# phecda-xu/FullyCNNSpeechEnhancement

Hardware: AMD Instinct MI355X
Metric: spectrogram frames/sec (CR-CED-16 fwd, 129-bin) (higher is better)
Workload: dtype f32; 1 GPU; CR-CED V3 (16-layer, skip connections) forward, batch 256 per GPU, 129x512, fp32 (BASELINE configs[2]); variant=FullyCNNV3, batch_per_gpu=256, frames=512, bins=129, global_batch=256, fused_available=True, parallelism=batch-shard x1, rccl_world_size=1, weights=random-init (glorot, seed 42), library=rced-hip 0.1 gfx950

## Files before the change

fullycnnspeechenhancement_amd/csrc/kernels_fused_v3_allx6.h:

```cpp
#pragma once

template <class M>
__device__ __forceinline__ void convert_px(unsigned lds0, int i, int f) {
  const unsigned src = lds0 + 4 * (M::kX0Off + 4 + i * kS + f);
  float v[8];
#pragma unroll
  for (int rr = 0; rr < 8; ++rr) v[rr] = lds_ld<float>(src, rr * kS * 4);
  u32x4 h, m, l;
#pragma unroll
  for (int q = 0; q < 4; ++q) {
    const P3 p = split2(v[2 * q], v[2 * q + 1]);
    h[q] = p.h;
    m[q] = p.m;
    l[q] = p.l;
  }
  const unsigned dst = lds0 + 4 * M::kB8Off + (kB8Pad + i * kS + f) * 16;
  lds_st<u32x4>(dst, 0, h);
  lds_st<u32x4>(dst, kB8PlaneBytes, m);
  lds_st<u32x4>(dst, 2 * kB8PlaneBytes, l);
}
template <class M>
__device__ __forceinline__ void convert_x0(unsigned lds0, int wave, int lane) {
  lane = opaque(lane);
  const int tid = wave * 64 + lane;
  convert_px<M>(lds0, tid >> 7, tid & 127);
  if (wave == 7 && lane < kTF) convert_px<M>(lds0, lane, kF - 1);
  const int z = tid - 5 * 64;
  if (z >= 0 && z < 72) {
    const int part = z / 24, rr = z - part * 24;
    const int row = rr < 4 ? rr : rr < 20 ? kB8Pad + kS * ((rr - 4) >> 2) + kF + ((rr - 4) & 3) : kB8Pad + kNPX + (rr - 20);
    lds_st<u32x4>(lds0 + 4 * M::kB8Off + part * kB8PlaneBytes + row * 16, 0, u32x4{0u, 0u, 0u, 0u});
  }
}
static_assert(kB8Rows == kB8Pad + kNPX + 4, "convert_x0 zeroes the planes' pad, gap and trailing rows by this map");

template <class M, int NCH, bool CT2ALL>
__device__ __forceinline__ void fin_run(unsigned ra, unsigned ta, int b0, int b2, int q0, bool ct2first, unsigned zaddr, f32x4 (&acc)[3]) {
  s16x8 a[2][3];
  Parts b[2][3];
  auto ld = [&](auto ic) {
    constexpr int i = decltype(ic)::value, r = i & 1;
    const int q = q0 + i;
    const unsigned ta_i = ta + (unsigned)(64 * q);
#pragma unroll
    for (int p = 0; p < 3; ++p) a[r][p] = lds_ld<s16x8>(ta_i, p * kFinTPart);
    const unsigned ra_i = ra + (unsigned)(16 * (4 * q + (q >> 2)));
    const int bq = b0 + 4 * q;
#pragma unroll
    for (int ct = 0; ct < 3; ++ct) {
      if (ct == 2 && !(CT2ALL || i == 0)) continue;
      const bool ok = ct < 2 ? (unsigned)(bq + 64 * ct) <= 128u : (unsigned)(b2 + 4 * q) <= 128u;
      const unsigned ad = ok ? ra_i + 1088u * ct : zaddr;
      b[r][ct].h = lds_ld<s16x8>(ad, 0);
      b[r][ct].m = lds_ld<s16x8>(ad, kHPlaneBytes);
      b[r][ct].l = lds_ld<s16x8>(ad, 2 * kHPlaneBytes);
    }
  };
  ld(IC<0>{});
  pin();
  static_for<0, NCH>([&](auto ic) {
    constexpr int i = decltype(ic)::value, r = i & 1;
    if constexpr (i + 1 < NCH) ld(IC<i + 1>{});
    pin();
    mma2(a[r], b[r][0], acc[0], a[r], b[r][1], acc[1]);
    if constexpr (CT2ALL) {
      acc[2] = l2x_mma(a[r], b[r][2], acc[2]);
    } else if constexpr (i == 0) {
      if (ct2first) acc[2] = l2x_mma(a[r], b[r][2], acc[2]);
    }
    pin();
  });
}

template <class M>
__device__ __forceinline__ void final_phase_x6(const Params& P, unsigned lds0, int wave, int lane, int utt, int t0, const XStage& xnext, float* x0 DET_ARG) {
  DET_BEGIN();
  lane = opaque(lane);
  const int n = lane & 15, kq = lane >> 4;
  const f32x4 zero4 = {0.f, 0.f, 0.f, 0.f};
  float* yt = P.y + ((size_t)utt * P.T + t0) * kF;
  const int nfr = P.T - t0 < kTF ? P.T - t0 : kTF;
  xstage_store(xnext, x0, wave * 64 + lane);
  {
    const int fi = n >> 2, j0 = n & 3;
    const int b0 = 16 * j0 - 64 + kq;
    const int b2 = j0 == 0 ? b0 + 128 : 0x40000000;
    const unsigned ra = lds0 + 4 * M::kB8Off + (unsigned)((kHFr * fi + 17 * j0 - 68 + kq) * 16);
    const unsigned ta = lds0 + 4 * M::kFinTOff + (unsigned)((kq - n + 15) * 16);
    const unsigned zaddr = lds0 + 4 * M::kB8Off + kHZeroRow * 16;
    f32x4 acc[3] = {zero4, zero4, zero4};
    if (wave < 4) {
      fin_run<M, 4, true>(ra, ta, b0, b2, 4 * wave, false, zaddr, acc);
    } else {
      const int run = 11 - wave;
      fin_run<M, 5, false>(ra, ta, b0, b2, 16 + 5 * (run - 4), run == 4, zaddr, acc);
    }
    const unsigned scr = lds0 + (unsigned)M::finscr(wave, 0) + (unsigned)lane * 16u;
#pragma unroll
    for (int ct = 0; ct < 3; ++ct) lds_st<f32x4>(scr, ct * M::kPlaneBytes, acc[ct]);
  }
  DET(8);
  __syncthreads();
  DET(9);
  if (wave < 3) {
    const unsigned scr = lds0 + (unsigned)(M::finscr(0, 0) + wave * M::kPlaneBytes) + (unsigned)lane * 16u;
    f32x4 v = lds_ld<f32x4>(scr, 0);
#pragma unroll
    for (int w = 1; w < kWaves; ++w) v += lds_ld<f32x4>(scr, M::finscr(w, 0) - M::finscr(0, 0));
    v += f32x4{P.fin_bias, P.fin_bias, P.fin_bias, P.fin_bias};
    const int fi = n >> 2;
    if (wave < 2) {
      const int f0 = 16 * (4 * wave + (n & 3)) + 4 * kq;
      if (fi < nfr) {
        *reinterpret_cast<f32x4_u*>(yt + fi * kF + f0) = v;
        store_wait_state();
      }
    } else if (kq == 0 && (n & 3) == 0 && fi < nfr) {
      yt[fi * kF + kF - 1] = v.x;
    }
  }
  DET(10);
  convert_x0<M>(lds0, wave, lane);
  DET(11);
  __syncthreads();
  DET(12);
}
```

fullycnnspeechenhancement_amd/csrc/kernels_fused_v3_l23.h:

```cpp
#pragma once
#ifndef RCED_T_A2REG
#define RCED_T_A2REG 3
#endif
#ifndef RCED_T_PRIO
#define RCED_T_PRIO 1
#endif
#ifndef RCED_T_TAILW
#define RCED_T_TAILW 4
#endif
#ifndef RCED_T_A3D
#define RCED_T_A3D 1
#endif
#ifndef RCED_T_SGB
#define RCED_T_SGB 1
#endif
#ifndef RCED_T_L1PF
#define RCED_T_L1PF 1
#endif
#ifndef RCED_T_EXP
#define RCED_T_EXP 0
#endif
#if (RCED_T_EXP != 0 || RCED_X6_EXP != 0) && !defined(RCED_TIMING_ONLY)
#error "RCED_T_EXP / RCED_X6_EXP builds compute wrong results: timing experiments only (tools/mkexp.sh ... -DRCED_TIMING_ONLY -DRCED_T_EXP=...)"
#endif

template <int CTRL>
__device__ __forceinline__ float dpp0(float v) {
  return __builtin_bit_cast(float, __builtin_amdgcn_update_dpp(0, __builtin_bit_cast(int, v), CTRL, 0xf, 0xf, true));
}
template <int S>
__device__ __forceinline__ void tap_add(float p, float& oP, float& oC, float& oN) {
  if constexpr (S == 0) {
    oC += p;
  } else if constexpr (S > 0) {
    oC += dpp0<0x110 + S>(p);
    oN += dpp0<0x100 + 16 - S>(p);
  } else {
    oC += dpp0<0x100 - S>(p);
    oP += dpp0<0x110 + 16 + S>(p);
  }
}
__device__ __forceinline__ void mma2(const s16x8 (&a0)[3], const Parts& b0, f32x4& c0, const s16x8 (&a1)[3], const Parts& b1, f32x4& c1) {
  c0 = mfma32(a0[1], b0.m, c0);
  c1 = mfma32(a1[1], b1.m, c1);
  c0 = mfma32(a0[2], b0.h, c0);
  c1 = mfma32(a1[2], b1.h, c1);
  c0 = mfma32(a0[0], b0.l, c0);
  c1 = mfma32(a1[0], b1.l, c1);
  c0 = mfma32(a0[1], b0.h, c0);
  c1 = mfma32(a1[1], b1.h, c1);
  c0 = mfma32(a0[0], b0.m, c0);
  c1 = mfma32(a1[0], b1.m, c1);
  c0 = mfma32(a0[0], b0.h, c0);
  c1 = mfma32(a1[0], b1.h, c1);
}
template <int NM, int NV, int ND = 0>
__device__ __forceinline__ void interleave() {
#if RCED_T_SGB
#pragma unroll
  for (int i = 0; i < NM; ++i) {
    __builtin_amdgcn_sched_group_barrier(0x008, 1, 0);
    if (ND > 0) __builtin_amdgcn_sched_group_barrier(0x100, ND, 0);
    __builtin_amdgcn_sched_group_barrier(0x002, NV, 0);
  }
#endif
}
template <int J>
__device__ __forceinline__ void shift_add(f32x4 pj, float& p0, float& p1, float& c0, float& c1, float& n0, float& n1) {
  if (RCED_T_EXP & 1) {
    c0 += pj.x;
    c1 += pj.z;
    return;
  }
  tap_add<4 - 2 * J>(pj.x, p0, c0, n0);
  if constexpr (2 * J + 1 < 9) tap_add<3 - 2 * J>(pj.y, p0, c0, n0);
  tap_add<4 - 2 * J>(pj.z, p1, c1, n1);
  if constexpr (2 * J + 1 < 9) tap_add<3 - 2 * J>(pj.w, p1, c1, n1);
}

template <class M>
struct MapTag {
  typedef M type;
};
template <class M>
constexpr int tail_off() {
  if constexpr (M::kAllX6) return M::kTailOff;
  else return 0;
}
template <class M, bool LAST, class Sp, class Dma1>
__device__ __forceinline__ void layer23(const Params& P, const Lane& L, unsigned lds0, unsigned wbase, const A2Regs& A, int blk, int wave,
                                        unsigned tag, f32x2 (&sk1)[5], f32x2 (&sk2)[5], Sp sp, Dma1 dma1 DET_ARG) {
  DET_BEGIN();
  const bool right = wave >= 4;
  const int fr = wave & 3;
  const unsigned a2 = wbase + L.scr, a3 = a2 + kG2 * 4;
  const f32x4 sh2[2] = {lds_ld<f32x4>(wbase + L.kq16, kG2Data * 4), lds_ld<f32x4>(wbase + L.kq16, (kG2Data + 16) * 4)};
  const f32x2 sh3 = lds_ld<f32x2>(wbase + (L.kq16 >> 1), (kG2 + kW3TData) * 4);
  const f32x4 zero4 = {0.f, 0.f, 0.f, 0.f};
  const f32x2 zero2 = {0.f, 0.f};
  Parts b2[2];
  s16x8 a2m0[3][3];
  if constexpr (RCED_T_A2REG == 3) {
#pragma unroll
    for (int c = 0; c < 3; ++c)
#pragma unroll
      for (int q = 0; q < 3; ++q) a2m0[c][q] = lds_ld<s16x8>(a2, ((2 * c) * 3 + q) * 1024);
  }
  s16x8 a2r[2][2][3];
  unsigned rdc = L.rd2c;
  f32x4 acc2[2][2];
  u32x4 b3h[2], b3m[2], b3l[2];
  s16x8 a3r[RCED_T_A3D + 1][3];
  f32x4 pj[2][2], p4[2] = {zero4, zero4};
  float w0 = -0.f, w1 = -0.f, x0 = -0.f, x1 = -0.f, y0 = -0.f, y1 = -0.f, z0 = -0.f, z1 = -0.f;
  f32x2 hold = zero2;

  auto ldX = [&](auto tc, auto cc) {
    constexpr int t = decltype(tc)::value, c = decltype(cc)::value;
    if ((RCED_T_EXP & 8) && (c > 0 || t > 1)) return;
    Parts& b = b2[(3 * t + c) & 1];
#pragma unroll
    for (int mt = (RCED_T_A2REG == 3 ? 1 : RCED_T_A2REG); mt < 2; ++mt)
#pragma unroll
      for (int q = 0; q < 3; ++q) a2r[(3 * t + c) & 1][mt][q] = lds_ld<s16x8>(a2, ((2 * c + mt) * 3 + q) * 1024);
    if constexpr (c < 2) {
      constexpr int off = t * M::kTileB18 + (M::kAllX6 ? 32 : 64) * c;
      b.h = lds_ld<s16x8>(L.rd2m, off);
      b.m = lds_ld<s16x8>(L.rd2m, off + M::kPlaneBytes);
      b.l = lds_ld<s16x8>(L.rd2m, off + 2 * M::kPlaneBytes);
    } else {
      u32x4 h, m, l;
#pragma unroll
      for (int i = 0; i < 4; ++i) {
        h[i] = lds_ld<unsigned>(rdc, 4 * i);
        m[i] = lds_ld<unsigned>(rdc, 4 * i + M::kPlaneBytes);
        l[i] = lds_ld<unsigned>(rdc, 4 * i + 2 * M::kPlaneBytes);
      }
      b.h = __builtin_bit_cast(s16x8, h);
      b.m = __builtin_bit_cast(s16x8, m);
      b.l = __builtin_bit_cast(s16x8, l);
      rdc += L.rd2cs;
    }
  };
  auto doX = [&](auto tc, auto cc) {
    constexpr int t = decltype(tc)::value, c = decltype(cc)::value, r = (3 * t + c) & 1, u = t & 1;
    if constexpr (c == 0) {
      acc2[u][0] = sh2[0];
      acc2[u][1] = sh2[1];
    }
    mma2(RCED_T_A2REG == 3 ? a2m0[c] : RCED_T_A2REG >= 1 ? A.a[0][c] : a2r[r][0], b2[r], acc2[u][0], RCED_T_A2REG == 2 ? A.a[1][c] : a2r[r][1], b2[r], acc2[u][1]);
  };
  auto split_piece = [&](auto tc, auto qc) {
    constexpr int t = decltype(tc)::value, q = decltype(qc)::value, u = t & 1, mt = q >> 1;
    float v0 = relu1((q & 1) ? acc2[u][mt].z : acc2[u][mt].x), v1 = relu1((q & 1) ? acc2[u][mt].w : acc2[u][mt].y);
    if constexpr (t == 4) {
      const bool ok = vbit(L, kVN0);
      v0 = ok ? v0 : 0.f;
      v1 = ok ? v1 : 0.f;
    }
    P3 p;
    if (RCED_T_EXP & 4) {
      p.h = __builtin_bit_cast(unsigned, v0);
      p.m = __builtin_bit_cast(unsigned, v1);
      p.l = p.h;
    } else {
      p = split2(v0, v1);
    }
    b3h[u][q] = p.h;
    b3m[u][q] = p.m;
    b3l[u][q] = p.l;
  };
  auto ldY = [&](auto jc, auto parc) {
    constexpr int j = decltype(jc)::value, r = (j + decltype(parc)::value) % (RCED_T_A3D + 1);
    if ((RCED_T_EXP & 2) && j > 1) return;
#pragma unroll
    for (int q = 0; q < 3; ++q) a3r[r][q] = lds_ld<s16x8>(a3, (((RCED_T_EXP & 32) ? 0 : j) * 3 + ((RCED_T_EXP & 64) ? 0 : q)) * 1024);
  };
  auto doY = [&](auto uc, auto jc, auto parc) {
    constexpr int u = decltype(uc)::value, j = decltype(jc)::value, r = (j + decltype(parc)::value) % (RCED_T_A3D + 1);
    Parts b;
    b.h = __builtin_bit_cast(s16x8, b3h[u]);
    b.m = __builtin_bit_cast(s16x8, b3m[u]);
    b.l = __builtin_bit_cast(s16x8, b3l[u]);
    if constexpr (j == kL3MT - 1) p4[u] = l2x_mma(a3r[r], b, zero4);
    else pj[u][j & 1] = l2x_mma(a3r[r], b, zero4);
  };
  auto doYY = [&](auto jc, auto parc) {
    constexpr int j = decltype(jc)::value, r = (j + decltype(parc)::value) % (RCED_T_A3D + 1);
    Parts ba, bb;
    ba.h = __builtin_bit_cast(s16x8, b3h[0]);
    ba.m = __builtin_bit_cast(s16x8, b3m[0]);
    ba.l = __builtin_bit_cast(s16x8, b3l[0]);
    bb.h = __builtin_bit_cast(s16x8, b3h[1]);
    bb.m = __builtin_bit_cast(s16x8, b3m[1]);
    bb.l = __builtin_bit_cast(s16x8, b3l[1]);
    f32x4 ca = zero4, cb = zero4;
    mma2(a3r[r], ba, ca, a3r[r], bb, cb);
    if constexpr (j == kL3MT - 1) {
      p4[0] = ca;
      p4[1] = cb;
    } else {
      pj[0][j & 1] = ca;
      pj[1][j & 1] = cb;
    }
  };
  auto finish = [&](auto tc, float s0, float s1) {
    constexpr int t = decltype(tc)::value;
    f32x2 v = {relu1(s0 + sh3.x), relu1(s1 + sh3.y)};
    if constexpr (LAST) {
      v += sk1[t];
    } else {
      v += blk == 3 ? sk2[t] : zero2;
      sk1[t] = blk == 0 ? v : sk1[t];
      sk2[t] = blk == 1 ? v : sk2[t];
    }
    if constexpr (M::kAllX6 && LAST) {
      const P3 p = split2(v.x, v.y);
      if (t < 4 || vbit(L, kVN0)) {
        lds_st<unsigned>(L.wh0, t * 272, p.h);
        lds_st<unsigned>(L.wh0, t * 272 + kHPlaneBytes, p.m);
        lds_st<unsigned>(L.wh0, t * 272 + 2 * kHPlaneBytes, p.l);
      }
    } else if constexpr (RCED_T_L1X6 && !LAST) {
      const P3 p = split2(v.x, v.y);
      if (t < 4 || vbit(L, kVN0)) {
        lds_st<unsigned>(L.wr3p, t * 256, p.h);
        lds_st<unsigned>(L.wr3p, t * 256 + kB8PlaneBytes, p.m);
        lds_st<unsigned>(L.wr3p, t * 256 + 2 * kB8PlaneBytes, p.l);
      }
    } else {
      if (t < 4 || vbit(L, kVN0)) lds_st<f32x2>(LAST ? L.wh0 : L.wr3, t * (16 * kB8S * 4), v);
    }
  };
  static_assert(kHS == kB8S, "one tile stride for both destinations");
  const unsigned edge = lds0 + 4 * M::kEdgeOff + fr * 1024 + L.a8, eflag = lds0 + 4 * M::kEdgeFlagOff + fr * 8;
  auto publish = [&](int dir, float v0, float v1) {
    lds_st<f32x2>(edge, dir * 512, f32x2{v0, v1});
    cbar();
    if (L.a4 == 0) lds_poke_a(eflag + dir * 4, tag);
  };
  auto fetch = [&](int dir) {
    flag_wait(eflag + dir * 4, tag, P.err, 8u);
    return lds_ld<f32x2>(edge, dir * 512);
  };
  auto tail_pair = [&](auto ac) {
    constexpr int a = decltype(ac)::value;
    shift_add<4>(p4[0], w0, w1, x0, x1, y0, y1);
    shift_add<4>(p4[1], x0, x1, y0, y1, z0, z1);
    if constexpr (a == 0) {
      if (right) {
        publish(1, w0, w1);
        hold = f32x2{x0, x1};
      } else {
        finish(IC<0>{}, x0, x1);
      }
    } else {
      finish(IC<a - 1>{}, w0, w1);
      finish(IC<a>{}, x0, x1);
    }
    w0 = y0;
    w1 = y1;
    x0 = z0;
    x1 = z1;
    y0 = y1 = z0 = z1 = -0.f;
  };
  auto runX = [&](auto tc, auto nc, auto prev_tail) {
    constexpr int t = decltype(tc)::value, next = decltype(nc)::value;
    static_for<0, 3>([&](auto cc) {
      constexpr int c = decltype(cc)::value;
      if constexpr (c < 2) ldX(tc, IC<c + 1>{});
      else if constexpr (next == 0) ldX(IC<t + 1>{}, IC<0>{});
      if constexpr (next == 1 && c + RCED_T_A3D >= 3) ldY(IC<c + RCED_T_A3D - 3>{}, IC<0>{});
      if (RCED_T_SGB < 2) pin();
      doX(tc, cc);
      if constexpr (c == 0) prev_tail();
      if constexpr (t > 0) {
        if constexpr (c == 0) {
          split_piece(IC<t - 1>{}, IC<0>{});
          split_piece(IC<t - 1>{}, IC<1>{});
        } else if constexpr (c == 1) {
          split_piece(IC<t - 1>{}, IC<2>{});
          split_piece(IC<t - 1>{}, IC<3>{});
        }
      }
      interleave<12, (c == 0 ? 5 : 3), (RCED_T_SGB >= 2 ? 2 : 0)>();
      pin();
    });
  };
  auto runY = [&](auto ac, auto pairc, auto nc, auto nxc, auto parc, auto prev_tail) {
    constexpr int a = decltype(ac)::value, next = decltype(nc)::value, u0 = a & 1;
    constexpr bool pair = decltype(pairc)::value != 0;
    static_for<0, kL3MT>([&](auto jc) {
      constexpr int j = decltype(jc)::value;
      constexpr int D = RCED_T_A3D, par = decltype(parc)::value, npar = (kL3MT + par) % (D + 1);
      if constexpr (j + D < kL3MT) ldY(IC<j + D>{}, parc);
      else if constexpr (next == 1) ldY(IC<j + D - kL3MT>{}, IC<npar>{});
      if constexpr (next == 0 && j == kL3MT - 1) ldX(nxc, IC<0>{});
      if (RCED_T_SGB < 2) pin();
      if constexpr (pair) doYY(jc, parc);
      else doY(IC<u0>{}, jc, parc);
      if constexpr (j == 0) {
        prev_tail();
      } else {
        shift_add<j - 1>(pj[u0][(j - 1) & 1], w0, w1, x0, x1, y0, y1);
        if constexpr (pair) shift_add<j - 1>(pj[u0 ^ 1][(j - 1) & 1], x0, x1, y0, y1, z0, z1);
      }
      if constexpr (next == 2) sp(jc);
      interleave<(pair ? 12 : 6), (j == 0 ? 4 : 2), (RCED_T_SGB >= 2 ? 1 : 0)>();
      pin();
    });
  };
  auto none = [] {};
  const IC<0> i0;
  const IC<1> i1;
  const IC<2> i2;
  const IC<3> i3;
  const IC<4> i4;

  const int tln = (int)(L.a4 >> 2), tn = tln & 15, tkq = tln >> 4, tf = tn & 3;
  const unsigned tb = lds0 + 4 * tail_off<M>();
  constexpr int kT3 = 2 * 3 * 16 * 8, kTFlag = kT3 + 4 * 5 * 4 * 8;
  auto tail2 = [&](auto mapc, int mt) {
    using MA = typename decltype(mapc)::type;
    const unsigned PL = lds0 + 4 * MA::kB18Off, px = kS * tf + 64;
    const unsigned rm = PL + (tkq & 1) * MA::kHalfBytes + (px + (tkq >> 1)) * 16;
    const unsigned rc = tkq < 2 ? rm + 64 + 4 * MA::kTileB18 : PL + MA::kRemOff + (px + 4 * (tkq & 1)) * 4 + 4 * 64;
    const unsigned am = a2 + (unsigned)mt * 3072u;
    f32x4 acc = mt ? sh2[1] : sh2[0];
    static_for<0, 3>([&](auto cc) {
      constexpr int c = decltype(cc)::value;
      Parts b;
      if constexpr (c < 2) {
        b.h = lds_ld<s16x8>(rm, 4 * MA::kTileB18 + 32 * c);
        b.m = lds_ld<s16x8>(rm, 4 * MA::kTileB18 + 32 * c + MA::kPlaneBytes);
        b.l = lds_ld<s16x8>(rm, 4 * MA::kTileB18 + 32 * c + 2 * MA::kPlaneBytes);
      } else {
        u32x4 h, m, l;
#pragma unroll
        for (int i = 0; i < 4; ++i) {
          h[i] = lds_ld<unsigned>(rc, 4 * i);
          m[i] = lds_ld<unsigned>(rc, 4 * i + MA::kPlaneBytes);
          l[i] = lds_ld<unsigned>(rc, 4 * i + 2 * MA::kPlaneBytes);
        }
        b.h = __builtin_bit_cast(s16x8, h);
        b.m = __builtin_bit_cast(s16x8, m);
        b.l = __builtin_bit_cast(s16x8, l);
      }
      s16x8 a[3];
#pragma unroll
      for (int q = 0; q < 3; ++q) a[q] = lds_ld<s16x8>(am, (6 * c + q) * 1024);
      acc = l2x_mma(a, b, acc);
    });
    const P3 p0 = split2(relu1(acc.x), relu1(acc.y)), p1 = split2(relu1(acc.z), relu1(acc.w));
    const unsigned r = tb + (unsigned)(mt * 3 * 16 + tkq * 4 + tf) * 8u;
    lds_st<u32x2>(r, 0, u32x2{p0.h, p1.h});
    lds_st<u32x2>(r, 16 * 8, u32x2{p0.m, p1.m});
    lds_st<u32x2>(r, 32 * 8, u32x2{p0.l, p1.l});
    cbar();
    if (L.a4 == 0) lds_poke_a(tb + kTFlag + 4 * mt, tag);
  };
  auto tail3 = [&](auto j0c, auto j1c) {
    constexpr int j0 = decltype(j0c)::value, j1 = decltype(j1c)::value;
    flag_wait(tb + kTFlag, tag, P.err, 8u);
    flag_wait(tb + kTFlag + 4, tag, P.err, 8u);
    const unsigned r = tb + (unsigned)(tkq * 4 + tf) * 8u;
    Parts b;
    const u32x2 h0 = lds_ld<u32x2>(r, 0), m0 = lds_ld<u32x2>(r, 16 * 8), l0 = lds_ld<u32x2>(r, 32 * 8);
    const u32x2 h1 = lds_ld<u32x2>(r, 48 * 8), m1 = lds_ld<u32x2>(r, 64 * 8), l1 = lds_ld<u32x2>(r, 80 * 8);
    b.h = __builtin_bit_cast(s16x8, u32x4{h0[0], h0[1], h1[0], h1[1]});
    b.m = __builtin_bit_cast(s16x8, u32x4{m0[0], m0[1], m1[0], m1[1]});
    b.l = __builtin_bit_cast(s16x8, u32x4{l0[0], l0[1], l1[0], l1[1]});
    static_for<j0, j1>([&](auto jc) {
      constexpr int j = decltype(jc)::value;
      s16x8 a[3];
#pragma unroll
      for (int q = 0; q < 3; ++q) a[q] = lds_ld<s16x8>(a3, (j * 3 + q) * 1024);
      const f32x4 p = l2x_mma(a, b, zero4);
      const unsigned o = tb + kT3 + (unsigned)((tf * 5 + 2 * j - 4) * 4 + tkq) * 8u;
      lds_st<f32x2>(o, 0, f32x2{p.x, p.z});
      if constexpr (2 * j + 1 < 9) lds_st<f32x2>(o, 32, f32x2{p.y, p.w});
    });
    cbar();
    if (L.a4 == 0) lds_poke_a(tb + kTFlag + 8 + 4 * (j0 == 2 ? 0 : 1), tag);
  };
  const bool tail = M::kAllX6 && !(RCED_T_EXP & 1024);

  if (RCED_T_PRIO && right) __builtin_amdgcn_s_setprio(RCED_T_PRIO);
  const int tw = wave - RCED_T_TAILW;
  if constexpr (M::kAllX6) {
    if (tail && (tw == 0 || tw == 1)) tail2(MapTag<M>{}, tw);
  }
  ldX(i0, i0);
  pin();
  if (!(RCED_T_EXP & 512)) dma1();
  pin();
  runX(i0, i0, none);
  if constexpr (M::kAllX6) {
    if (tail && tw == 2) tail3(i2, i4);
    else if (tail && tw == 3) tail3(i4, IC<5>{});
  }
  runX(i1, i0, none);
  runX(i2, i1, none);
  DET(0);
  runY(i0, i1, i0, i3, i0, none);
  DET(1);
  if (!right) {
    runX(i3, i1, [&] { tail_pair(i0); });
    DET(2);
    static_for<0, 4>([&](auto qc) { split_piece(i3, qc); });
    runY(i2, i1, i2, i0, i0, none);
    tail_pair(i2);
    publish(0, x0, x1);
    const f32x2 e = fetch(1);
    finish(i3, w0 + e.x, w1 + e.y);
  } else if (M::kAllX6) {
    runX(i3, i1, [&] { tail_pair(i0); });
    DET(2);
    static_for<0, 4>([&](auto qc) { split_piece(i3, qc); });
    runY(i2, i1, i2, i0, i0, none);
    tail_pair(i2);
    if (tail) {
      flag_wait(tb + kTFlag + 8, tag, P.err, 8u);
      flag_wait(tb + kTFlag + 12, tag, P.err, 8u);
      const int ti = tn >= 12 ? 16 - tn : 0;
      const f32x2 r = lds_ld<f32x2>(tb + kT3 + (unsigned)((fr * 5 + ti) * 4 + tkq) * 8u, 0);
      if (tn >= 12) {
        w0 += r.x;
        w1 += r.y;
      } else if (tn == 0) {
        x0 += r.x;
        x1 += r.y;
      }
    }
    finish(i3, w0, w1);
    finish(i4, x0, x1);
    const f32x2 e = fetch(0);
    finish(i0, hold.x + e.x, hold.y + e.y);
    if (RCED_T_PRIO) __builtin_amdgcn_s_setprio(0);
  } else {
    runX(i3, i0, [&] { tail_pair(i0); });
    runX(i4, i1, none);
    DET(2);
    runY(i2, i1, i1, i0, i0, none);
    static_for<0, 4>([&](auto qc) { split_piece(i4, qc); });
    runY(i4, i0, i2, i0, IC<kL3MT % (RCED_T_A3D + 1)>{}, [&] { tail_pair(i2); });
    shift_add<4>(p4[0], w0, w1, x0, x1, y0, y1);
    finish(i3, w0, w1);
    finish(i4, x0, x1);
    const f32x2 e = fetch(0);
    finish(i0, hold.x + e.x, hold.y + e.y);
    if (RCED_T_PRIO) __builtin_amdgcn_s_setprio(0);
  }
  DET(3);
}


__device__ __forceinline__ Parts b8_load(unsigned rd, int off) {
  Parts b;
  b.h = lds_ld<s16x8>(rd, off);
  if (RCED_T_EXP & 256) {
    b.m = b.l = b.h;
    return b;
  }
  b.m = lds_ld<s16x8>(rd, off + kB8PlaneBytes);
  b.l = lds_ld<s16x8>(rd, off + 2 * kB8PlaneBytes);
  return b;
}

template <class M>
constexpr int a1x_off(int i) {
  if constexpr (M::kAllX6) return M::kW1Off * 4 + i * 1024;
  else return i < 5 ? M::kX0Off * 4 + i * 1024
                    : M::kHOff * 4 + (kHFrame * ((i - 5) / 4) + 64) * kHS * 4 + 8 * (((i - 5) / 4) & 1) + ((i - 5) % 4) * 1024;
}
template <class M>
constexpr int a1x_shift_off() {
  if constexpr (M::kAllX6) return M::kW1Off * 4 + kG1APieces * 1024;
  else return M::kX0Off * 4 + 5 * 1024;
}
#if RCED_V3_LEGACY_FORMS
static_assert(a1x_shift_off<MapT>() + 128 <= (MapT::kX0Off + kX0Floats) * 4 && a1x_off<MapT>(20) + 1024 <= (MapT::kHOff + (kHFrame * 3 + 64 + kF) * kHS) * 4 &&
              a1x_off<MapT>(8) % 16 == 0 && a1x_off<MapT>(9) % 16 == 0 && a1x_off<MapT>(13) % 16 == 0 && a1x_off<MapT>(17) % 16 == 0,
              "layer 1's LDS-resident images: inside the input-row area / the real bins of the H image, 16-byte aligned");
#endif
template <class M>
__device__ __forceinline__ void a1x_dma(const float* src, float* lds, int wave, int lane) {
  constexpr int kPieces = M::kAllX6 ? kG1APieces : 21;
  lane = opaque(lane);
#pragma unroll
  for (int k = 0; k < 3; ++k) {
    const int ci = wave + 8 * k;
    if (ci < kPieces) {
      lds_dma16s(src + ci * 256, (unsigned)lane * 16u, lds + a1x_off<M>(ci) / 4);
    } else if (ci == kPieces) {
      if (lane < 8) lds_dma16s(src + kPieces * 256, (unsigned)lane * 16u, lds + a1x_shift_off<M>() / 4);
    }
  }
}
template <class M, int I>
__device__ __forceinline__ s16x8 a1x_ld(unsigned aX, unsigned aH) {
  if constexpr (I < 5 || M::kAllX6) return lds_ld<s16x8>(aX, I * 1024);
  else return lds_ld<s16x8>(aH, a1x_off<M>(I) - M::kHOff * 4);
}
template <class M, class Dma, class Sp>
__device__ __forceinline__ void layer1_x6l(const Lane& L, unsigned lds0, int role, Dma dma, Sp sp DET_ARG) {
  DET_BEGIN();
  constexpr int kTW = M::kT1W, kTR = 128 * 16;
  const unsigned aX = lds0 + (M::kAllX6 ? a1x_off<M>(0) : M::kX0Off * 4) + L.scr, aH = lds0 + M::kHOff * 4 + L.scr;
  const f32x4 sh = lds_ld<f32x4>(lds0 + a1x_shift_off<M>() + L.kq16, 0);
  const f32x2 s2 = lds_ld<f32x2>(lds0 + a1x_shift_off<M>(), 64);
  auto pre = once(dma);
  auto lda = [&](auto pc, s16x8 (&a)[3]) {
    constexpr int g = decltype(pc)::value;
    a[0] = a1x_ld<M, 3 * g>(aX, aH);
    a[1] = a1x_ld<M, 3 * g + 1>(aX, aH);
    a[2] = a1x_ld<M, 3 * g + 2>(aX, aH);
  };
  constexpr bool kPF = M::kAllX6 && RCED_T_L1PF;
  constexpr bool kFold = M::kAllX6;
  constexpr int kRemPiece = kFold ? 8 : 9;
  auto ldar = [&](auto cc, s16x8 (&a)[3]) {
    constexpr int c = decltype(cc)::value;
    a[0] = a1x_ld<M, kRemPiece + 3 * c>(aX, aH);
    a[1] = a1x_ld<M, kRemPiece + 3 * c + 1>(aX, aH);
    a[2] = a1x_ld<M, kRemPiece + 3 * c + 2>(aX, aH);
  };
  const bool has_single = role < 2 || role == 7, has_rem = role >= 4;
  const unsigned rd_single = L.rd1x + (role == 0 ? 32 : role == 1 ? 30 : 16) * 256;
  Parts nb;
  s16x8 na[3];
  auto prefetch = [&](unsigned rd, int aoff) {
    nb = b8_load(rd, 0);
#pragma unroll
    for (int q = 0; q < 3; ++q) na[q] = lds_ld<s16x8>(aX + aoff, q * 1024);
  };
  if constexpr (kFold) {
    Parts b[2][2];
    s16x8 bf[2];
    s16x8 a[2][3], af[2];
    f32x4 acc[2][2];
    const bool two = role != 7;
    const bool g1 = tile_has_gap(role + 8), g2 = tile_has_gap(role + 16), g3 = tile_has_gap(role + 24);
    auto ld = [&](auto ic) {
      constexpr int i = decltype(ic)::value, p = i / 2, c = i % 2;
      if constexpr (p == 0) lda(IC<c>{}, a[c]);
      b[c][0] = b8_load(L.rd1x, 2 * p * kTR + 64 * c);
      b[c][1] = b8_load(L.rd1xb, 2 * p * kTR + 64 * c);
      if constexpr (c == 1) {
        if constexpr (p == 0) {
          af[0] = a1x_ld<M, 6>(aX, aH);
          af[1] = a1x_ld<M, 7>(aX, aH);
        }
        if (RCED_T_EXP & 32768) return;
        bf[0] = lds_ld<s16x8>(L.rd1f, 2 * p * kTR);
        bf[1] = lds_ld<s16x8>(L.rd1f, 2 * p * kTR + 128 * 16);
      }
    };
    auto slot = [&](auto ic) {
      constexpr int i = decltype(ic)::value, p = i / 2, c = i % 2;
      if constexpr (c == 0) acc[p][0] = acc[p][1] = sh;
      mma2(a[c], b[c][0], acc[p][0], a[c], b[c][1], acc[p][1]);
      if (c == 1 && !(RCED_T_EXP & 32768)) {
        acc[p][0] = mfma32(af[0], bf[0], acc[p][0]);
        acc[p][1] = mfma32(af[0], bf[1], acc[p][1]);
        acc[p][0] = mfma32(af[1], bf[0], acc[p][0]);
        acc[p][1] = mfma32(af[1], bf[1], acc[p][1]);
      }
      if constexpr (p == 0) static_for<0, (c == 0 ? 4 : 5)>([&](auto qc) { sp(IC<12 + 4 * c + decltype(qc)::value>{}); });
      if constexpr (i == 2) l1_store<M>(L, acc[0][0], L.wr1, 0, false, kVMain);
      if constexpr (i == 3) l1_store<M>(L, acc[0][1], L.wr1, kTW, g1, kVMain + 1);
      interleave<(c == 1 && !(RCED_T_EXP & 32768) ? 16 : 12), 3>();
    };
    ld(IC<0>{});
    pin();
    if (!(RCED_T_EXP & 512)) pre();
    pin();
    static_for<0, 2>([&](auto ic) {
      constexpr int i = decltype(ic)::value;
      if constexpr (i < 1) ld(IC<i + 1>{});
      else if (two) ld(IC<2>{});
      pin();
      slot(ic);
      pin();
      DETX(i);
    });
    if (two) {
      static_for<2, 4>([&](auto ic) {
        constexpr int i = decltype(ic)::value;
        if constexpr (i < 3) ld(IC<i + 1>{});
        pin();
        slot(ic);
        pin();
        DETX(i);
      });
      if constexpr (kPF) {
        if (has_single) prefetch(rd_single, 0);
        else if (has_rem) prefetch(L.rd1xr, kRemPiece * 1024);
        pin();
      }
      l1_store<M>(L, acc[1][0], L.wr1, 2 * kTW, g2, kVMain + 2);
      l1_store<M>(L, acc[1][1], L.wr1, 3 * kTW, g3, kVMain + 3);
      DETX(6);
    } else {
      if constexpr (kPF) {
        prefetch(rd_single, 0);
        pin();
      }
      l1_store<M>(L, acc[0][0], L.wr1, 0, false, 0);
      l1_store<M>(L, acc[0][1], L.wr1, kTW, false, 0);
    }
  } else {
    Parts b[2][2];
    s16x8 a[3][3];
    f32x4 acc[2][2];
    const bool two = role != 7;
    const bool g1 = tile_has_gap(role + 8), g2 = tile_has_gap(role + 16), g3 = tile_has_gap(role + 24);
    auto ld = [&](auto ic) {
      constexpr int i = decltype(ic)::value, p = i / 3, c = i % 3;
      if constexpr (p == 0) lda(IC<c>{}, a[c]);
      b[i & 1][0] = b8_load(L.rd1x, 2 * p * kTR + 64 * c);
      b[i & 1][1] = b8_load(L.rd1xb, 2 * p * kTR + 64 * c);
    };
    auto slot = [&](auto ic) {
      constexpr int i = decltype(ic)::value, p = i / 3, c = i % 3;
      if constexpr (c == 0) acc[p][0] = acc[p][1] = sh;
      mma2(a[c], b[i & 1][0], acc[p][0], a[c], b[i & 1][1], acc[p][1]);
      if constexpr (p == 0) static_for<0, 3>([&](auto qc) { sp(IC<12 + 3 * i + decltype(qc)::value>{}); });
      if constexpr (p == 1 && c == 0) l1_store<M>(L, acc[0][0], L.wr1, 0, false, kVMain);
      if constexpr (p == 1 && c == 1) l1_store<M>(L, acc[0][1], L.wr1, kTW, g1, kVMain + 1);
      interleave<12, 3>();
    };
    ld(IC<0>{});
    pin();
    if (!(RCED_T_EXP & 512)) pre();
    pin();
    static_for<0, 3>([&](auto ic) {
      constexpr int i = decltype(ic)::value;
      if constexpr (i < 2) ld(IC<i + 1>{});
      else if (two) ld(IC<3>{});
      pin();
      slot(ic);
      pin();
      DETX(i);
    });
    if (two) {
      static_for<3, 6>([&](auto ic) {
        constexpr int i = decltype(ic)::value;
        if constexpr (i < 5) ld(IC<i + 1>{});
        pin();
        slot(ic);
        pin();
        DETX(i);
      });
      if constexpr (kPF) {
        if (has_single) prefetch(rd_single, 0);
        else if (has_rem) prefetch(L.rd1xr, kRemPiece * 1024);
        pin();
      }
      l1_store<M>(L, acc[1][0], L.wr1, 2 * kTW, g2, kVMain + 2);
      l1_store<M>(L, acc[1][1], L.wr1, 3 * kTW, g3, kVMain + 3);
      DETX(6);
    } else {
      if constexpr (kPF) {
        prefetch(rd_single, 0);
        pin();
      }
      l1_store<M>(L, acc[0][0], L.wr1, 0, false, 0);
      l1_store<M>(L, acc[0][1], L.wr1, kTW, false, 0);
    }
  }
  DET(6);
  if (RCED_T_EXP & 8192) return;
  if (role < 2 || role == 7) {
    const int dt = role == 0 ? 32 : role == 1 ? 30 : 16;
    const unsigned rd = L.rd1x + dt * 256;
    Parts b[2];
    s16x8 a[2][3];
    f32x4 acc = sh;
    if constexpr (kPF) {
      b[0] = nb;
      a[0][0] = na[0];
      a[0][1] = na[1];
      a[0][2] = na[2];
    } else {
      b[0] = b8_load(rd, 0);
      lda(IC<0>{}, a[0]);
    }
    pin();
    static_for<0, 3>([&](auto cc) {
      constexpr int c = decltype(cc)::value;
      if constexpr (kFold && c == 1) {
        if (!(RCED_T_EXP & 32768)) b[0].h = lds_ld<s16x8>(L.rd1f + dt * 256, 0);
        a[0][0] = a1x_ld<M, 6>(aX, aH);
        a[0][1] = a1x_ld<M, 7>(aX, aH);
      } else if constexpr (c < 2) {
        b[(c + 1) & 1] = b8_load(rd, 64 * (c + 1));
        lda(IC<c + 1>{}, a[(c + 1) & 1]);
      }
      pin();
      if ((RCED_T_EXP & 32768) && c == 2) {
      } else if constexpr (kFold && c == 2) {
        acc = mfma32(a[0][0], b[0].h, acc);
        acc = mfma32(a[0][1], b[0].h, acc);
      } else {
        acc = l2x_mma(a[c & 1], b[c & 1], acc);
      }
      pin();
    });
    if constexpr (kPF) {
      if (has_rem) prefetch(L.rd1xr, kRemPiece * 1024);
      pin();
    }
    l1_store<M>(L, acc, L.wr1 + dt * M::kTileB18, 0, false, 0);
  }
  DET(5);
  {
    const int nrem = role < 4 ? 0 : role == 7 ? 2 : 1;
    unsigned rdr = L.rd1xr, wrr = L.wr1r;
    int xr = role == 7 ? 3 : role - 4, vb = kVRem;
    const f32x4 init = {s2.x, s2.y, s2.x, s2.y};
#pragma unroll 1
    for (int r = 0; r < nrem; ++r) {
      Parts b[2];
      s16x8 a[2][3];
      f32x4 acc = init;
      if (kPF && r == 0) {
        b[0] = nb;
        a[0][0] = na[0];
        a[0][1] = na[1];
        a[0][2] = na[2];
      } else {
        b[0] = b8_load(rdr, 0);
        ldar(IC<0>{}, a[0]);
      }
      pin();
      static_for<0, 4>([&](auto cc) {
        constexpr int c = decltype(cc)::value;
        if constexpr (c < 3) {
          b[(c + 1) & 1] = b8_load(rdr, 64 * (c + 1));
          ldar(IC<c + 1>{}, a[(c + 1) & 1]);
        }
        pin();
        acc = l2x_mma(a[c & 1], b[c & 1], acc);
        pin();
      });
      const f32x4 v = relu4(acc);
      const bool va = xr == 0 || vbit(L, vb), vbb = vbit(L, vb + 1);
      const P3 pa = split2(v.x, v.y), pb = split2(v.z, v.w);
      if (va) {
        lds_st<unsigned>(wrr, 0, pa.h);
        lds_st<unsigned>(wrr, M::kPlaneBytes, pa.m);
        lds_st<unsigned>(wrr, 2 * M::kPlaneBytes, pa.l);
      }
      if (vbb) {
        lds_st<unsigned>(wrr, 4, pb.h);
        lds_st<unsigned>(wrr, M::kPlaneBytes + 4, pb.m);
        lds_st<unsigned>(wrr, 2 * M::kPlaneBytes + 4, pb.l);
      }
      wrr += 112 * 4;
      rdr += 112 * 16;
      xr += 1;
      vb += 2;
    }
  }
  DET(4);
}
```

Measured before the change: 23.88 million frames/s.

## Spread tail split-precision MFMA planes across lane groups with DPP reduction

The tail2/tail3 stages now let each group of 4 lanes (tpart) load a single precision plane (h/m/l) instead of every lane loading all three planes and running the full split-precision MMA. Per-plane partial products come from plain mfma32 calls and are combined across lane groups with a DPP group_sum, and only lanes tn<4 write results. A-operand loads in tail3 are hoisted above the flag wait. This is meant to cut LDS loads and MFMA count in the tail path, at the cost of extra DPP shuffles and a changed tail buffer layout. It also adds an RCED_X6_EXP&32 timing switch that skips ct2 in the final phase.

Result: no change. 24.05 million frames/s, median of 6 (+0.7%).

```diff
diff --git a/fullycnnspeechenhancement_amd/csrc/kernels_fused_v3_allx6.h b/fullycnnspeechenhancement_amd/csrc/kernels_fused_v3_allx6.h
--- a/fullycnnspeechenhancement_amd/csrc/kernels_fused_v3_allx6.h
+++ b/fullycnnspeechenhancement_amd/csrc/kernels_fused_v3_allx6.h
@@ -48,7 +48,7 @@
     const int bq = b0 + 4 * q;
 #pragma unroll
     for (int ct = 0; ct < 3; ++ct) {
-      if (ct == 2 && !(CT2ALL || i == 0)) continue;
+      if (ct == 2 && (!(CT2ALL || i == 0) || (RCED_X6_EXP & 32))) continue;
       const bool ok = ct < 2 ? (unsigned)(bq + 64 * ct) <= 128u : (unsigned)(b2 + 4 * q) <= 128u;
       const unsigned ad = ok ? ra_i + 1088u * ct : zaddr;
       b[r][ct].h = lds_ld<s16x8>(ad, 0);
@@ -63,7 +63,8 @@
     if constexpr (i + 1 < NCH) ld(IC<i + 1>{});
     pin();
     mma2(a[r], b[r][0], acc[0], a[r], b[r][1], acc[1]);
-    if constexpr (CT2ALL) {
+    if constexpr (RCED_X6_EXP & 32) {
+    } else if constexpr (CT2ALL) {
       acc[2] = l2x_mma(a[r], b[r][2], acc[2]);
     } else if constexpr (i == 0) {
       if (ct2first) acc[2] = l2x_mma(a[r], b[r][2], acc[2]);
diff --git a/fullycnnspeechenhancement_amd/csrc/kernels_fused_v3_l23.h b/fullycnnspeechenhancement_amd/csrc/kernels_fused_v3_l23.h
--- a/fullycnnspeechenhancement_amd/csrc/kernels_fused_v3_l23.h
+++ b/fullycnnspeechenhancement_amd/csrc/kernels_fused_v3_l23.h
@@ -320,65 +320,71 @@
   const int tln = (int)(L.a4 >> 2), tn = tln & 15, tkq = tln >> 4, tf = tn & 3;
   const unsigned tb = lds0 + 4 * tail_off<M>();
   constexpr int kT3 = 2 * 3 * 16 * 8, kTFlag = kT3 + 4 * 5 * 4 * 8;
+  const int tg = tn >> 2;
+  const unsigned tpart = tg < 3 ? (unsigned)tg : 0u;
+  auto group_sum = [&](f32x4 v) {
+    f32x4 r;
+#pragma unroll
+    for (int i = 0; i < 4; ++i) {
+      const float t = v[i] + dpp0<0x104>(v[i]);
+      r[i] = v[i] + dpp0<0x104>(t);
+    }
+    return r;
+  };
   auto tail2 = [&](auto mapc, int mt) {
     using MA = typename decltype(mapc)::type;
-    const unsigned PL = lds0 + 4 * MA::kB18Off, px = kS * tf + 64;
+    const unsigned PL = lds0 + 4 * MA::kB18Off + tpart * MA::kPlaneBytes, px = kS * tf + 64;
     const unsigned rm = PL + (tkq & 1) * MA::kHalfBytes + (px + (tkq >> 1)) * 16;
     const unsigned rc = tkq < 2 ? rm + 64 + 4 * MA::kTileB18 : PL + MA::kRemOff + (px + 4 * (tkq & 1)) * 4 + 4 * 64;
     const unsigned am = a2 + (unsigned)mt * 3072u;
-    f32x4 acc = mt ? sh2[1] : sh2[0];
-    static_for<0, 3>([&](auto cc) {
-      constexpr int c = decltype(cc)::value;
-      Parts b;
-      if constexpr (c < 2) {
-        b.h = lds_ld<s16x8>(rm, 4 * MA::kTileB18 + 32 * c);
-        b.m = lds_ld<s16x8>(rm, 4 * MA::kTileB18 + 32 * c + MA::kPlaneBytes);
-        b.l = lds_ld<s16x8>(rm, 4 * MA::kTileB18 + 32 * c + 2 * MA::kPlaneBytes);
-      } else {
-        u32x4 h, m, l;
-#pragma unroll
-        for (int i = 0; i < 4; ++i) {
-          h[i] = lds_ld<unsigned>(rc, 4 * i);
-          m[i] = lds_ld<unsigned>(rc, 4 * i + MA::kPlaneBytes);
-          l[i] = lds_ld<unsigned>(rc, 4 * i + 2 * MA::kPlaneBytes);
-        }
-        b.h = __builtin_bit_cast(s16x8, h);
-        b.m = __builtin_bit_cast(s16x8, m);
-        b.l = __builtin_bit_cast(s16x8, l);
-      }
-      s16x8 a[3];
-#pragma unroll
-      for (int q = 0; q < 3; ++q) a[q] = lds_ld<s16x8>(am, (6 * c + q) * 1024);
-      acc = l2x_mma(a, b, acc);
-    });
+    s16x8 b[3], a[3][3];
+    b[0] = lds_ld<s16x8>(rm, 4 * MA::kTileB18);
+    b[1] = lds_ld<s16x8>(rm, 4 * MA::kTileB18 + 32);
+    u32x4 bc;
+#pragma unroll
+    for (int i = 0; i < 4; ++i) bc[i] = lds_ld<unsigned>(rc, 4 * i);
+    b[2] = __builtin_bit_cast(s16x8, bc);
+#pragma unroll
+    for (int c = 0; c < 3; ++c)
+#pragma unroll
+      for (int q = 0; q < 3; ++q) a[c][q] = lds_ld<s16x8>(am, (6 * c + q) * 1024);
+    f32x4 s[3] = {zero4, zero4, zero4};
+#pragma unroll
+    for (int c = 0; c < 3; ++c)
+#pragma unroll
+      for (int q = 2; q >= 0; --q) s[q] = mfma32(a[c][q], b[c], s[q]);
+    const f32x4 acc = group_sum((s[2] + s[1]) + s[0]) + (mt ? sh2[1] : sh2[0]);
     const P3 p0 = split2(relu1(acc.x), relu1(acc.y)), p1 = split2(relu1(acc.z), relu1(acc.w));
-    const unsigned r = tb + (unsigned)(mt * 3 * 16 + tkq * 4 + tf) * 8u;
-    lds_st<u32x2>(r, 0, u32x2{p0.h, p1.h});
-    lds_st<u32x2>(r, 16 * 8, u32x2{p0.m, p1.m});
-    lds_st<u32x2>(r, 32 * 8, u32x2{p0.l, p1.l});
+    if (tn < 4) {
+      const unsigned r = tb + (unsigned)(tkq * 4 + tf) * 16u + (unsigned)mt * 8u;
+      lds_st<u32x2>(r, 0, u32x2{p0.h, p1.h});
+      lds_st<u32x2>(r, 256, u32x2{p0.m, p1.m});
+      lds_st<u32x2>(r, 512, u32x2{p0.l, p1.l});
+    }
     cbar();
     if (L.a4 == 0) lds_poke_a(tb + kTFlag + 4 * mt, tag);
   };
   auto tail3 = [&](auto j0c, auto j1c) {
     constexpr int j0 = decltype(j0c)::value, j1 = decltype(j1c)::value;
+    s16x8 a[j1 - j0][3];
+    static_for<j0, j1>([&](auto jc) {
+      constexpr int j = decltype(jc)::value;
+#pragma unroll
+      for (int q = 0; q < 3; ++q) a[j - j0][q] = lds_ld<s16x8>(a3, (j * 3 + q) * 1024);
+    });
     flag_wait(tb + kTFlag, tag, P.err, 8u);
     flag_wait(tb + kTFlag + 4, tag, P.err, 8u);
-    const unsigned r = tb + (unsigned)(tkq * 4 + tf) * 8u;
-    Parts b;
-    const u32x2 h0 = lds_ld<u32x2>(r, 0), m0 = lds_ld<u32x2>(r, 16 * 8), l0 = lds_ld<u32x2>(r, 32 * 8);
-    const u32x2 h1 = lds_ld<u32x2>(r, 48 * 8), m1 = lds_ld<u32x2>(r, 64 * 8), l1 = lds_ld<u32x2>(r, 80 * 8);
-    b.h = __builtin_bit_cast(s16x8, u32x4{h0[0], h0[1], h1[0], h1[1]});
-    b.m = __builtin_bit_cast(s16x8, u32x4{m0[0], m0[1], m1[0], m1[1]});
-    b.l = __builtin_bit_cast(s16x8, u32x4{l0[0], l0[1], l1[0], l1[1]});
+    const s16x8 b = lds_ld<s16x8>(tb + (unsigned)((tpart * 4 + tkq) * 4 + tf) * 16u, 0);
     static_for<j0, j1>([&](auto jc) {
       constexpr int j = decltype(jc)::value;
-      s16x8 a[3];
-#pragma unroll
-      for (int q = 0; q < 3; ++q) a[q] = lds_ld<s16x8>(a3, (j * 3 + q) * 1024);
-      const f32x4 p = l2x_mma(a, b, zero4);
-      const unsigned o = tb + kT3 + (unsigned)((tf * 5 + 2 * j - 4) * 4 + tkq) * 8u;
-      lds_st<f32x2>(o, 0, f32x2{p.x, p.z});
-      if constexpr (2 * j + 1 < 9) lds_st<f32x2>(o, 32, f32x2{p.y, p.w});
+      f32x4 p = mfma32(a[j - j0][2], b, zero4);
+      p = mfma32(a[j - j0][1], b, p);
+      p = group_sum(mfma32(a[j - j0][0], b, p));
+      if (tn < 4) {
+        const unsigned o = tb + kT3 + (unsigned)((tf * 5 + 2 * j - 4) * 4 + tkq) * 8u;
+        lds_st<f32x2>(o, 0, f32x2{p.x, p.z});
+        if constexpr (2 * j + 1 < 9) lds_st<f32x2>(o, 32, f32x2{p.y, p.w});
+      }
     });
     cbar();
     if (L.a4 == 0) lds_poke_a(tb + kTFlag + 8 + 4 * (j0 == 2 ? 0 : 1), tag);
```
